# Zhen-Dong/HAWQ

Hardware: NVIDIA H100
Metric: images/sec ResNet-50 W8A8 & W4A4 @batch128, 1/2/4/8xH100; % int-TC roofline (higher is better)
Workload: dtype int8

## Files before the change

hawq_b200/csrc/api.cu:

```cuda
#include <cmath>
#include <cstdarg>
#include <cstdio>
#include <cstring>

#include <cstdlib>

#include "conv_igemm.cuh"
#include "conv_tail.cuh"
#include "elementwise.cuh"
#include "eval_transform.cuh"
#include "mobilenet.cuh"
#include "stem.cuh"

using namespace hawq;

struct hawq_handle {
  int device;
  int sm_count;
  int32_t* status;
};

static thread_local char g_err[512] = "";
static long long g_kernel_count[8] = {0, 0, 0, 0, 0, 0, 0, 0};

namespace hawq {
int fail(int code, const char* fmt, ...) {
  va_list ap;
  va_start(ap, fmt);
  vsnprintf(g_err, sizeof(g_err), fmt, ap);
  va_end(ap);
  return code;
}
}

#define CUDA_TRY(expr)                                                                         \
  do {                                                                                         \
    cudaError_t _e = (expr);                                                                   \
    if (_e != cudaSuccess) return fail(HAWQ_ERR_CUDA, "%s: %s", #expr, cudaGetErrorString(_e)); \
  } while (0)

static int launch_check(const char* what) {
  cudaError_t e = cudaGetLastError();
  if (e != cudaSuccess) return fail(HAWQ_ERR_CUDA, "%s launch: %s", what, cudaGetErrorString(e));
  return HAWQ_OK;
}

static int grid_for(long long work_items, int sm_count) {
  long long blocks = (work_items + 255) / 256;
  const long long cap = (long long)sm_count * 16;
  if (blocks > cap) blocks = cap;
  if (blocks < 1) blocks = 1;
  return (int)blocks;
}

template <class K>
static int set_smem_attr(K* kernel, int smem) {
  CUDA_TRY(cudaFuncSetAttribute(kernel, cudaFuncAttributeMaxDynamicSharedMemorySize, smem));
  CUDA_TRY(cudaFuncSetAttribute(kernel, cudaFuncAttributePreferredSharedMemoryCarveout, cudaSharedmemCarveoutMaxShared));
  return HAWQ_OK;
}
template <int BN, bool A4>
static int set_conv_attr() {
  constexpr int smem = ConvSmem<BN, A4>::TOTAL;
  int rc;
  if ((rc = set_smem_attr(conv_igemm_kernel<BN, A4, FAM_REQUANT>, smem)) || (rc = set_smem_attr(conv_igemm_kernel<BN, A4, FAM_RESIDUAL>, smem)) ||
      (rc = set_smem_attr(conv_igemm_kernel<BN, A4, FAM_REQUANT_CAPPED>, smem)) ||
      (rc = set_smem_attr(conv_igemm_kernel<BN, A4, FAM_STORE>, smem)) ||
      (rc = set_smem_attr(conv_tail_kernel<A4, false>, TailSmem<A4, false>::TOTAL)) ||
      (rc = set_smem_attr(conv_tail_kernel<A4, true>, TailSmem<A4, true>::TOTAL)))
    return rc;
  return HAWQ_OK;
}

static dim3 conv_grid(long long M, int Cout, int BN) { return dim3((unsigned)((M + CONV_BM - 1) / CONV_BM * (Cout / BN)), 1, 1); }

template <int BN, bool A4>
static void launch_conv(const ConvParams& p, cudaStream_t s) {
  const int smem = ConvSmem<BN, A4>::TOTAL;
  const dim3 grid = conv_grid(p.M, p.Cout, BN);
  if (p.mode == HAWQ_EPI_REQUANT && p.relu == 2) conv_igemm_kernel<BN, A4, FAM_REQUANT_CAPPED><<<grid, CONV_THREADS, smem, s>>>(p);
  else if (p.mode == HAWQ_EPI_REQUANT) conv_igemm_kernel<BN, A4, FAM_REQUANT><<<grid, CONV_THREADS, smem, s>>>(p);
  else if (p.mode == HAWQ_EPI_RESIDUAL) conv_igemm_kernel<BN, A4, FAM_RESIDUAL><<<grid, CONV_THREADS, smem, s>>>(p);
  else conv_igemm_kernel<BN, A4, FAM_STORE><<<grid, CONV_THREADS, smem, s>>>(p);
}
template <bool A4, bool DUAL>
static void launch_conv_tail(const ConvParams& p, int sm_count, cudaStream_t s) {
  conv_tail_kernel<A4, DUAL><<<tail_grid(p.Cout, sm_count), CONV_THREADS, TailSmem<A4, DUAL>::TOTAL, s>>>(p);
}

extern "C" {

int hawq_abi_version(void) { return HAWQ_ABI_VERSION; }
const char* hawq_last_error(void) { return g_err; }

static int create_on(int device, hawq_handle** out) {
  CUDA_TRY(cudaSetDevice(device));
  cudaDeviceProp prop;
  CUDA_TRY(cudaGetDeviceProperties(&prop, device));
  if (prop.major != 9 || prop.minor != 0)
    return fail(HAWQ_ERR_UNSUPPORTED, "hawq_create: device sm_%d%d is not Hopper sm_90 (the library is built for sm_90a)", prop.major, prop.minor);
  hawq_handle* h = new hawq_handle();
  h->device = device;
  h->sm_count = prop.multiProcessorCount;
  h->status = nullptr;
  CUDA_TRY(cudaMalloc(&h->status, sizeof(int32_t)));
  CUDA_TRY(cudaMemset(h->status, 0, sizeof(int32_t)));
  int rc;
  CUDA_TRY(cudaFuncSetAttribute(linear_dp4a_kernel, cudaFuncAttributeMaxDynamicSharedMemorySize, linear_smem_bytes(LIN_MAX_K)));
  if ((rc = set_conv_attr<128, false>()) || (rc = set_conv_attr<64, false>()) || (rc = set_conv_attr<128, true>()) ||
      (rc = set_conv_attr<64, true>()))
    return rc;
  *out = h;
  return HAWQ_OK;
}

int hawq_create(int device, hawq_handle** out) {
  if (!out) return fail(HAWQ_ERR_BAD_ARG, "hawq_create: out is null");
  int prev = 0;
  CUDA_TRY(cudaGetDevice(&prev));
  int rc = create_on(device, out);
  cudaSetDevice(prev);
  return rc;
}

int hawq_destroy(hawq_handle* h) {
  if (!h) return HAWQ_OK;
  cudaFree(h->status);
  delete h;
  return HAWQ_OK;
}

int hawq_sm_count(const hawq_handle* h) { return h ? h->sm_count : 0; }

int hawq_reset_status(hawq_handle* h, void* stream) {
  if (!h) return fail(HAWQ_ERR_BAD_ARG, "null handle");
  CUDA_TRY(cudaMemsetAsync(h->status, 0, sizeof(int32_t), (cudaStream_t)stream));
  return HAWQ_OK;
}

int hawq_get_status(hawq_handle* h, void* stream, int32_t* host_flags) {
  if (!h || !host_flags) return fail(HAWQ_ERR_BAD_ARG, "null argument");
  CUDA_TRY(cudaMemcpyAsync(host_flags, h->status, sizeof(int32_t), cudaMemcpyDeviceToHost, (cudaStream_t)stream));
  CUDA_TRY(cudaStreamSynchronize((cudaStream_t)stream));
  return HAWQ_OK;
}

int hawq_copy_status(hawq_handle* h, int32_t* dst, void* stream) {
  if (!h || !dst) return fail(HAWQ_ERR_BAD_ARG, "null argument");
  CUDA_TRY(cudaMemcpyAsync(dst, h->status, sizeof(int32_t), cudaMemcpyDeviceToDevice, (cudaStream_t)stream));
  return HAWQ_OK;
}

static int check_me(const char* fn, const char* what, uint32_t m, int e) {
  return e < 1 || e > 62 || m > 0x80000000u ? fail(HAWQ_ERR_BAD_ARG, "%s: %s dyadic pair out of range (m=%u e=%d)", fn, what, m, e) : HAWQ_OK;
}

static int out_size(int in, int k, int stride, int pad) { return (in + 2 * pad - k) / stride + 1; }

static int check_conv_desc(const char* fn, const hawq_conv_desc* d, int bn) {
  if (d->N < 1 || d->H < 1 || d->W < 1 || d->kh < 1 || d->kw < 1 || d->stride < 1 || d->pad < 0) return fail(HAWQ_ERR_BAD_ARG, "%s: bad geometry", fn);
  if (d->a_bits != 8 && d->a_bits != 4) return fail(HAWQ_ERR_UNSUPPORTED, "%s: a_bits must be 4 or 8", fn);
  if (d->Cin % 64 != 0 || d->Cout % 64 != 0) return fail(HAWQ_ERR_UNSUPPORTED, "%s: Cin (%d) and Cout (%d) must be multiples of 64", fn, d->Cin, d->Cout);
  if (d->Cin < 64 || d->Cout < 64) return fail(HAWQ_ERR_BAD_ARG, "%s: Cin (%d) and Cout (%d) must be at least 64", fn, d->Cin, d->Cout);
  const int Ho = out_size(d->H, d->kh, d->stride, d->pad), Wo = out_size(d->W, d->kw, d->stride, d->pad);
  if (Ho < 1 || Wo < 1) return fail(HAWQ_ERR_BAD_ARG, "%s: empty output", fn);
  const long long M = (long long)d->N * Ho * Wo;
  if (M > 0x7fffff00ll || (long long)d->N * d->H * d->W > 0x7fffff00ll) return fail(HAWQ_ERR_UNSUPPORTED, "%s: too many pixels", fn);
  if ((M + CONV_BM - 1) / CONV_BM * (d->Cout / bn) > 0x7fffffffll) return fail(HAWQ_ERR_UNSUPPORTED, "%s: more than 2^31 - 1 output tiles", fn);
  return HAWQ_OK;
}

static int check_dims(const char* fn, int N, int H, int W, int C, int min_side = 1) {
  return N < 1 || H < min_side || W < min_side || C < 1 ? fail(HAWQ_ERR_BAD_ARG, "%s: bad geometry", fn) : HAWQ_OK;
}

static int check_limits(const char* fn, long long pixels, long long ctas) {
  if (pixels > 0x7fffff00ll) return fail(HAWQ_ERR_UNSUPPORTED, "%s: too many pixels", fn);
  if (ctas > 0x7fffffffll) return fail(HAWQ_ERR_UNSUPPORTED, "%s: more than 2^31 - 1 CTAs", fn);
  return HAWQ_OK;
}

static int check_clamp(const char* fn, int lo, int hi, int bits = 0) {
  if (lo > hi) return fail(HAWQ_ERR_BAD_ARG, "%s: empty clamp range", fn);
  if (bits && (lo < -(1 << (bits - 1)) || hi >= 1 << (bits - 1))) return fail(HAWQ_ERR_BAD_ARG, "%s: clamp must fit int%d", fn, bits);
  return HAWQ_OK;
}

static int check_low(const char* fn, int low_bits, uint32_t low_m, int low_e, const void* out_low) {
  if (low_bits != 0 && low_bits != 4 && low_bits != 8) return fail(HAWQ_ERR_BAD_ARG, "%s: low_bits must be 0/4/8", fn);
  if (!low_bits) return HAWQ_OK;
  if (!out_low) return fail(HAWQ_ERR_BAD_ARG, "%s: low_bits set but out_low is null", fn);
  return check_me(fn, "low-bit copy", low_m, low_e);
}

static int check_residual(const char* fn, const hawq_epilogue_desc* ep, const void* res, const hawq_chan* res_chan, const void* y,
                          const void* out_low) {
  if (!res) return fail(HAWQ_ERR_BAD_ARG, "%s: RESIDUAL needs res", fn);
  if (ep->res_kind != 0 && ep->res_kind != 1) return fail(HAWQ_ERR_BAD_ARG, "%s: res_kind must be 0/1", fn);
  if (ep->res_kind == 1 && !res_chan) return fail(HAWQ_ERR_BAD_ARG, "%s: res_kind 1 needs res_chan", fn);
  if (ep->res_kind == 0 && ep->res_bits != 16 && ep->res_bits != 32) return fail(HAWQ_ERR_BAD_ARG, "%s: res_bits must be 16/32", fn);
  if (int rc = ep->res_kind == 0 ? check_me(fn, "residual", ep->res_m, ep->res_e) : HAWQ_OK) return rc;
  if (ep->y_bits != 0 && ep->y_bits != 16 && ep->y_bits != 32) return fail(HAWQ_ERR_BAD_ARG, "%s: y_bits must be 0/16/32", fn);
  if (ep->y_bits == 16 && !ep->relu) return fail(HAWQ_ERR_BAD_ARG, "%s: uint16 residual stream requires relu", fn);
  if (ep->y_bits && !y) return fail(HAWQ_ERR_BAD_ARG, "%s: y_bits set but the stream pointer is null", fn);
  if (!ep->y_bits && !ep->low_bits) return fail(HAWQ_ERR_BAD_ARG, "%s: RESIDUAL with no output", fn);
  return check_low(fn, ep->low_bits, ep->low_m, ep->low_e, out_low);
}

static void set_bias_window(ConvParams& p, int a_bits) {
  long long bound = (long long)p.K * (a_bits == 4 ? 15 * 128 : 128 * 128);
  if (bound > 2147483648ll) bound = 2147483648ll;
  p.bias_lo = (int)(bound - 2147483648ll);
  p.bias_hi = (int)(2147483647ll - bound);
}

static ConvParams conv_params(const hawq_handle* h, const hawq_conv_desc& d, const void* x, const int8_t* w, const hawq_chan* chan,
                              void* out, bool depthwise = false) {
  ConvParams p;
  memset(&p, 0, sizeof(p));
  p.x = (const uint8_t*)x; p.w = w; p.chan = chan; p.out = out; p.status = h->status;
  p.N = d.N; p.H = d.H; p.W = d.W; p.Cin = d.Cin; p.Cout = d.Cout; p.KH = d.kh; p.KW = d.kw; p.stride = d.stride; p.pad = d.pad;
  p.Ho = out_size(d.H, d.kh, d.stride, d.pad); p.Wo = out_size(d.W, d.kw, d.stride, d.pad);
  p.M = (int)((long long)d.N * p.Ho * p.Wo); p.K = d.kh * d.kw * (depthwise ? 1 : d.Cin);
  p.cin_chunks = d.Cin / 64; p.x_pix_bytes = d.Cin * d.a_bits / 8;
  set_bias_window(p, d.a_bits);
  return p;
}

static void set_epilogue(ConvParams& p, const hawq_epilogue_desc& ep, bool writes_low) {
  p.mode = ep.mode; p.relu = ep.relu; p.out_bits = ep.out_bits; p.lo = ep.clamp_lo; p.hi = ep.clamp_hi;
  p.res_kind = ep.res_kind; p.res_bits = ep.res_bits; p.res_m = ep.res_m; p.res_e = ep.res_e;
  p.y_bits = ep.y_bits; p.low_bits = ep.low_bits; p.low_m = ep.low_m; p.low_e = ep.low_e; p.low_lo = ep.low_lo; p.low_hi = ep.low_hi;
  p.cout_store = ep.cout_store;
  const bool residual = ep.mode == HAWQ_EPI_RESIDUAL, scalar_res = residual && ep.res_kind == 0;
  const bool low_over_one = writes_low && ep.low_bits != 0 && !dyadic_is_fast(ep.low_m, ep.low_e);
  p.scalar_over_one = (scalar_res && !dyadic_is_fast(ep.res_m, ep.res_e)) || low_over_one;
  p.scalar_unchecked = (scalar_res && !dyadic_is_wide(ep.res_m, ep.res_e)) || low_over_one;
  p.check_ovf = residual && (ep.flags & (HAWQ_EP_RATIOS_LE_ONE | HAWQ_EP_RATIOS_LE_2P20)) != 0;
}

static int persistent_ctas(long long tiles, int sm_count) { return (int)(tiles < 4LL * sm_count ? tiles : 4LL * sm_count); }

int hawq_conv2d(hawq_handle* h, const hawq_conv_desc* d, const hawq_epilogue_desc* ep, const void* x, const int8_t* w,
                const hawq_chan* chan, const void* res, const hawq_chan* res_chan, const float* fscale, void* out,
                void* out_low, void* stream) {
  if (!h || !d || !ep || !x || !w || !chan) return fail(HAWQ_ERR_BAD_ARG, "hawq_conv2d: null argument");
  const bool bn128 = (d->Cout % 128 == 0);
  if (int rc = check_conv_desc(__func__, d, bn128 ? 128 : 64)) return rc;
  switch (ep->mode) {
    case HAWQ_EPI_REQUANT:
      if (!out) return fail(HAWQ_ERR_BAD_ARG, "hawq_conv2d: REQUANT needs out");
      if (ep->out_bits != 4 && ep->out_bits != 8 && ep->out_bits != 16 && ep->out_bits != 32)
        return fail(HAWQ_ERR_BAD_ARG, "hawq_conv2d: out_bits must be 4/8/16/32");
      if (int rc = check_clamp(__func__, ep->clamp_lo, ep->clamp_hi)) return rc;
      break;
    case HAWQ_EPI_RESIDUAL:
      if (int rc = check_residual(__func__, ep, res, res_chan, out, out_low)) return rc;
      break;
    case HAWQ_EPI_RAW_I32:
      if (!out) return fail(HAWQ_ERR_BAD_ARG, "hawq_conv2d: RAW_I32 needs out");
      break;
    case HAWQ_EPI_DEQUANT_F32:
      if (!out || !fscale) return fail(HAWQ_ERR_BAD_ARG, "hawq_conv2d: DEQUANT_F32 needs out and fscale");
      if (ep->cout_store < 1 || ep->cout_store > d->Cout) return fail(HAWQ_ERR_BAD_ARG, "hawq_conv2d: bad cout_store");
      break;
    default:
      return fail(HAWQ_ERR_BAD_ARG, "hawq_conv2d: unknown epilogue mode %d", ep->mode);
  }

  ConvParams p = conv_params(h, *d, x, w, chan, out);
  p.res = res; p.res_chan = res_chan; p.fscale = fscale; p.out_low = out_low;
  set_epilogue(p, *ep, ep->mode == HAWQ_EPI_RESIDUAL);
  ++g_kernel_count[0];
  cudaStream_t s = (cudaStream_t)stream;
  const bool tail = ep->mode == HAWQ_EPI_RESIDUAL && d->kh == 1 && d->kw == 1 && d->stride == 1 && d->pad == 0 && ep->res_kind == 0 &&
                    ep->res_bits == 16 && ep->y_bits == 16;
  if (tail) {
    if (d->a_bits == 8) launch_conv_tail<false, false>(p, h->sm_count, s);
    else launch_conv_tail<true, false>(p, h->sm_count, s);
  } else if (d->a_bits == 8) {
    if (bn128) launch_conv<128, false>(p, s);
    else launch_conv<64, false>(p, s);
  } else {
    if (bn128) launch_conv<128, true>(p, s);
    else launch_conv<64, true>(p, s);
  }
  return launch_check("conv_igemm");
}

int hawq_conv2d_dual(hawq_handle* h, const hawq_conv_desc* d, const hawq_epilogue_desc* ep, const void* x, const int8_t* w,
                     const hawq_chan* chan, const hawq_conv_desc* d2, const void* x2, const int8_t* w2, const hawq_chan* chan2,
                     void* out, void* out_low, void* stream) {
  if (!h || !d || !ep || !x || !w || !chan || !d2 || !x2 || !w2 || !chan2 || !out) return fail(HAWQ_ERR_BAD_ARG, "hawq_conv2d_dual: null argument");
  if (d->kh != 1 || d->kw != 1 || d->stride != 1 || d->pad != 0 || d2->kh != 1 || d2->kw != 1 || d2->pad != 0 || d2->stride < 1)
    return fail(HAWQ_ERR_UNSUPPORTED, "hawq_conv2d_dual: both convolutions must be 1x1 without padding (main stride 1)");
  int rc;
  if ((rc = check_conv_desc(__func__, d, 64))) return rc;
  if (d2->a_bits != d->a_bits || d2->Cout != d->Cout) return fail(HAWQ_ERR_UNSUPPORTED, "hawq_conv2d_dual: a_bits and Cout must be equal");
  if (d2->N != d->N || out_size(d2->H, 1, d2->stride, 0) != d->H || out_size(d2->W, 1, d2->stride, 0) != d->W)
    return fail(HAWQ_ERR_BAD_ARG, "hawq_conv2d_dual: the two convolutions have different output grids");
  if ((rc = check_conv_desc(__func__, d2, 64))) return rc;
  if (d->w_layout != 1 || d2->w_layout != 1) return fail(HAWQ_ERR_UNSUPPORTED, "hawq_conv2d_dual: weights must carry the re-tiled copy (w_layout 1)");
  if (ep->mode != HAWQ_EPI_RESIDUAL || !ep->relu || ep->y_bits != 16) return fail(HAWQ_ERR_UNSUPPORTED, "hawq_conv2d_dual: RESIDUAL + relu + uint16 stream only");
  if ((rc = check_low(__func__, ep->low_bits, ep->low_m, ep->low_e, out_low))) return rc;
  if (ep->low_bits && !dyadic_is_fast(ep->low_m, ep->low_e)) return fail(HAWQ_ERR_UNSUPPORTED, "hawq_conv2d_dual: low-bit ratio outside the fast range");
  if (!(ep->flags & (HAWQ_EP_RATIOS_LE_ONE | HAWQ_EP_RATIOS_LE_2P20))) return fail(HAWQ_ERR_UNSUPPORTED, "hawq_conv2d_dual: needs a ratio-range promise (flags)");

  ++g_kernel_count[4];
  ConvParams p = conv_params(h, *d, x, w, chan, out);
  const ConvParams id = conv_params(h, *d2, x2, w2, chan2, nullptr);
  p.x2 = id.x; p.w2 = id.w; p.H2 = id.H; p.W2 = id.W; p.stride2 = id.stride; p.cin_chunks2 = id.cin_chunks; p.x2_pix_bytes = id.x_pix_bytes;
  p.res_chan = chan2; p.out_low = out_low;
  const hawq_epilogue_desc e = {HAWQ_EPI_RESIDUAL, 1, 0, 0, 0, 1, 32, 0, 0, 16, ep->low_bits, ep->low_m, ep->low_e, ep->low_lo, ep->low_hi, 0, ep->flags};
  set_epilogue(p, e, true);

  cudaStream_t s = (cudaStream_t)stream;
  if (d->a_bits == 8) launch_conv_tail<false, true>(p, h->sm_count, s);
  else launch_conv_tail<true, true>(p, h->sm_count, s);
  return launch_check("conv_dual");
}

int hawq_conv2d_i8(hawq_handle* h, const hawq_conv_desc* d, const hawq_epilogue_desc* ep, const void* x,
                   const int8_t* w, const hawq_chan* chan, const void* res, const hawq_chan* res_chan,
                   const float* fscale, void* out, void* out_low, void* stream) {
  if (d && d->a_bits != 8) return fail(HAWQ_ERR_BAD_ARG, "hawq_conv2d_i8: a_bits must be 8");
  return hawq_conv2d(h, d, ep, x, w, chan, res, res_chan, fscale, out, out_low, stream);
}

int hawq_conv2d_i4(hawq_handle* h, const hawq_conv_desc* d, const hawq_epilogue_desc* ep, const void* x,
                   const int8_t* w, const hawq_chan* chan, const void* res, const hawq_chan* res_chan,
                   const float* fscale, void* out, void* out_low, void* stream) {
  if (d && d->a_bits != 4) return fail(HAWQ_ERR_BAD_ARG, "hawq_conv2d_i4: a_bits must be 4");
  return hawq_conv2d(h, d, ep, x, w, chan, res, res_chan, fscale, out, out_low, stream);
}

int hawq_linear_i8(hawq_handle* h, int32_t N, int32_t K, int32_t Cout, int32_t Cout_pad, const int8_t* x,
                   const int8_t* w, const hawq_chan* chan, const float* fscale, float* out, void* stream) {
  if (Cout < 1 || Cout > Cout_pad) return fail(HAWQ_ERR_BAD_ARG, "hawq_linear_i8: bad Cout/Cout_pad");
  if (!h || !x || !w || !chan || !fscale || !out || N < 1 || K < 1) return fail(HAWQ_ERR_BAD_ARG, "hawq_linear_i8: null argument or empty shape");
  static const bool dp4a_enabled = [] { const char* e = getenv("HAWQ_B200_LINEAR_DP4A"); return !(e && e[0] == '0'); }();
  if (dp4a_enabled && K % LIN_SLAB == 0 && K <= LIN_MAX_K && Cout_pad % LIN_CH == 0 && N <= 65535 * LIN_ROWS) {
    const dim3 grid((unsigned)(Cout_pad / LIN_CH), (unsigned)((N + LIN_ROWS - 1) / LIN_ROWS), 1);
    linear_dp4a_kernel<<<grid, 256, linear_smem_bytes(K), (cudaStream_t)stream>>>(x, w, chan, fscale, out, N, K, Cout);
    return launch_check("linear_dp4a");
  }
  const hawq_conv_desc d = {N, 1, 1, K, Cout_pad, 1, 1, 1, 0, 8, 0};
  hawq_epilogue_desc ep = {};
  ep.mode = HAWQ_EPI_DEQUANT_F32;
  ep.cout_store = Cout;
  return hawq_conv2d(h, &d, &ep, x, w, chan, nullptr, nullptr, fscale, out, nullptr, stream);
}

static ConvParams stem_params(hawq_handle* h, int N, int H, int W, const int8_t* x, const int8_t* w, const hawq_chan* chan,
                              const hawq_epilogue_desc& ep, void* out, void* out_low) {
  ConvParams p = conv_params(h, {N, H, W, 3, 64, 7, 7, 2, 3, 8, 0}, x, w, chan, out);
  p.out_low = out_low;
  set_epilogue(p, ep, true);
  return p;
}

int hawq_stem_conv_i8(hawq_handle* h, int32_t N, int32_t H, int32_t W, const int8_t* x, const int8_t* w,
                      const hawq_chan* chan, int32_t clamp_lo, int32_t clamp_hi, int16_t* out, void* stream) {
// ... 238 lines not shown
```

hawq_b200/csrc/conv_igemm.cuh:

```cuda
#pragma once
#include <type_traits>

#include "common.cuh"
#include "wgmma.cuh"

namespace hawq {

struct ConvParams {
  const uint8_t* x;
  const int8_t* w;
  const hawq_chan* chan;
  const void* res;
  const hawq_chan* res_chan;
  const float* fscale;
  void* out;
  void* out_low;
  int32_t* status;
  int N, H, W, Cin, Cout, KH, KW, stride, pad, Ho, Wo, M, K;
  int cin_chunks;
  int x_pix_bytes;
  int mode, relu, out_bits, lo, hi;
  int res_kind, res_bits;
  uint32_t res_m;
  int res_e;
// ... 125 lines not shown
    if (checked && count) {
      const double q = t - kMagic;
      ovf |= q > 2147483647.0 || q < -2147483648.0;
    }
    return __double2loint(t);
  }
};
struct RqExact {
  bool checked;
  bool ovf = false;
  __device__ static int32_t acc_bias(int32_t acc, double, int32_t bias) { return sat_add(acc, bias); }
  __device__ static int32_t of_i32(int32_t v) { return v; }
  __device__ static int32_t of_u16(uint32_t u) { return (int32_t)u; }
  __device__ int32_t term(int32_t v, double, uint32_t m, int32_t e, bool count) {
    const long long q = rhe_requant64(v, m, e);
    if (checked && count) ovf |= q > 2147483647ll || q < -2147483648ll;
    return sat_i32(q);
  }
};

struct RqPolicy {
  bool over_one;
  bool unchecked;
  bool clamped;
};

template <int BN, bool RESIDUAL, bool CAPS = false>
__device__ RqPolicy load_channel_block(const ConvParams& p, int n0, const ChanSmem<BN>& cs) {
  int over_one = p.scalar_over_one, unchecked = p.scalar_unchecked, bias_out = 0;
  const int tid = threadIdx.x;
  if (tid < BN) {
    hawq_chan c = p.chan[n0 + tid];
    if (CAPS) c.reserved = p.relu == 2 ? min(p.hi, c.reserved) : p.hi;
    cs.chan[tid] = c;
    cs.M[tid] = dyadic_to_double(c.m, c.e);
    cs.Cb[tid] = 4503601774854144.0 - (double)c.bias;
    bias_out = c.bias < p.bias_lo || c.bias > p.bias_hi;
    over_one |= !dyadic_is_fast(c.m, c.e);
    unchecked |= !dyadic_is_wide(c.m, c.e);
    if (RESIDUAL && p.res_kind == 1) {
      const hawq_chan rc = p.res_chan[n0 + tid];
      cs.rc[tid] = rc;
      cs.M1[tid] = dyadic_to_double(rc.m, rc.e);
      over_one |= !dyadic_is_fast(rc.m, rc.e);
      unchecked |= !dyadic_is_wide(rc.m, rc.e);
    }
  }
  RqPolicy pol;
  pol.over_one = __syncthreads_or(over_one) != 0;
  pol.unchecked = __syncthreads_or(unchecked) != 0;
  pol.clamped = __syncthreads_or(bias_out) != 0;
  return pol;
}

template <bool RESIDUAL, class F>
__device__ __forceinline__ void with_rq(const RqPolicy& pol, const ConvParams& p, F&& f) {
  const bool fp64 = !pol.over_one || (RESIDUAL && p.check_ovf && !pol.unchecked);
  if (!fp64) f(RqExact{RESIDUAL && p.check_ovf != 0});
  else if (pol.clamped) f(RqFp64<true>{RESIDUAL && pol.over_one});
  else f(RqFp64<false>{RESIDUAL && pol.over_one});
}

template <class Rq>
__device__ __forceinline__ int32_t residual_y(Rq& rq, int32_t res_term, int32_t acc, double cb, const int4& c, double M, bool ok,
                                              int32_t relu_floor) {
  return max(sat_add(res_term, rq.term(rq.acc_bias(acc, cb, c.x), M, c.y, c.z, ok)), relu_floor);
}
template <class Rq>
__device__ __forceinline__ int32_t residual_low(Rq& rq, int32_t y, double low_M, const ConvParams& p) {
  return clampi(rq.term(rq.of_i32(y), low_M, p.low_m, p.low_e, false), p.low_lo, p.low_hi);
}
__device__ __forceinline__ uint32_t stream16_pair(int32_t y0, int32_t y1, bool ok, int& ymax) {
  if (ok) ymax = max(ymax, max(y0, y1));
  return (uint32_t)min(y0, 65535) | ((uint32_t)min(y1, 65535) << 16);
}
__device__ __forceinline__ void residual_flags(const ConvParams& p, int ymax, bool ovf) {
  if (ymax > 65535) atomicOr(p.status, HAWQ_FLAG_RESIDUAL_OVERFLOW);
  if (ovf) atomicOr(p.status, HAWQ_FLAG_REQUANT_OVERFLOW);
}
__device__ __forceinline__ void stage_low_pair(uint8_t* s, int pitch, int row, int col, int q0, int q1) {
  *reinterpret_cast<uint16_t*>(s + row * pitch + col) = (uint16_t)__byte_perm(q0, q1, 0x0040);
}

__device__ __forceinline__ void copy_out_rows(const uint8_t* s, int s_pitch, uint8_t* g, size_t g_pitch, int row_bytes, int m0, int M) {
  const int cpr = row_bytes / 16;
  for (int id = threadIdx.x; id < CONV_BM * cpr; id += blockDim.x) {
    const int row = id / cpr, j = id - row * cpr;
    if (m0 + row < M)
      *reinterpret_cast<int4*>(g + (size_t)(m0 + row) * g_pitch + j * 16) = *reinterpret_cast<const int4*>(s + row * s_pitch + j * 16);
  }
}
template <int BN>
__device__ __forceinline__ void copy_out_low(const uint8_t* s, int pitch, uint8_t* gout, int bits, int m0, int n0, int M, int Cout) {
  if (bits == 8) {
    copy_out_rows(s, pitch, gout + n0, (size_t)Cout, BN, m0, M);
  } else {
    constexpr int CPR = BN / 32;
    for (int id = threadIdx.x; id < CONV_BM * CPR; id += blockDim.x) {
      const int row = id / CPR, j = id % CPR;
      if (m0 + row < M) {
        const uint4 a = *reinterpret_cast<const uint4*>(s + row * pitch + j * 32);
        const uint4 b = *reinterpret_cast<const uint4*>(s + row * pitch + j * 32 + 16);
        uint4 o;
        o.x = pack_nibbles8(a.x, a.y);
        o.y = pack_nibbles8(a.z, a.w);
        o.z = pack_nibbles8(b.x, b.y);
        o.w = pack_nibbles8(b.z, b.w);
        *reinterpret_cast<uint4*>(gout + (((size_t)(m0 + row) * Cout + n0 + j * 32) >> 1)) = o;
      }
    }
  }
}

struct ConvGeom {
  const uint8_t* x;
  const int8_t* w;
  int H, W, stride, pad, KH, KW, cin_chunks, x_pix_bytes, K;
};

template <int BN, bool A4, int FAM>
__global__ void __launch_bounds__(CONV_THREADS, 2) conv_igemm_kernel(const ConvParams p) {
  using S = ConvSmem<BN, A4>;
  constexpr int BM = CONV_BM, STAGES = CONV_STAGES;
  constexpr int A_ROW = S::A_ROW, A_CH = S::A_CH, A_ROWS_PER_PASS = S::A_ROWS_PER_PASS, A_PASSES = S::A_PASSES;
  constexpr int NT = S::NT, NACC = S::NACC;
  constexpr int B_PASSES = BN / 64;

  extern __shared__ __align__(1024) uint8_t smem[];
  uint8_t* sA = smem;
  uint8_t* sB = smem + STAGES * S::A_STAGE;
  const ChanSmem<BN> cs(smem + S::CHAN_OFF);
  const hawq_chan* sChan = cs.chan;
  const double* sM = cs.M;
  const double* sM1 = cs.M1;
  const hawq_chan* sResChan = cs.rc;
  const double* sCb = cs.Cb;

  const int tid = threadIdx.x;
  const AccFrag fr(tid);
  const int nblk = p.Cout / BN;
  const int m0 = (int)(blockIdx.x / nblk) * BM;
  const int n0 = (int)(blockIdx.x % nblk) * BN;

  constexpr bool REQ = FAM == FAM_REQUANT || FAM == FAM_REQUANT_CAPPED;
  const RqPolicy pol = load_channel_block<BN, FAM == FAM_RESIDUAL, FAM == FAM_REQUANT_CAPPED>(p, n0, cs);

  int32_t acc[NACC];

  const int res_es = (FAM == FAM_RESIDUAL) ? ((p.res_kind == 1 || p.res_bits == 32) ? 4 : 2) : 0;
  const int res_pitch = tile_pitch(BN, res_es);
  uint8_t* sRes = smem + (res_es == 2 ? S::RES16_OFF : S::RES32_OFF);

  auto load_res = [&]() {
    if constexpr (FAM == FAM_RESIDUAL) load_res_tile<BN>(sRes, p, res_es, m0, n0);
  };
  const bool prefetch_res = res_es == 2;

  auto gemm = [&](const ConvGeom& gm, bool with_res) {
#pragma unroll
    for (int i = 0; i < NACC; ++i) acc[i] = 0;
    const int a_ch = tid % A_CH;
    int a_hi0[A_PASSES], a_wi0[A_PASSES], a_pix[A_PASSES];
    bool a_ok[A_PASSES];
#pragma unroll
    for (int i = 0; i < A_PASSES; ++i) {
      const int row = tid / A_CH + i * A_ROWS_PER_PASS;
      const int m = m0 + row;
      a_ok[i] = m < p.M;
      const int mm = a_ok[i] ? m : 0;
      const int n = mm / (p.Ho * p.Wo);
      const int r = mm - n * (p.Ho * p.Wo);
      const int ho = r / p.Wo, wo = r - ho * p.Wo;
      a_hi0[i] = ho * gm.stride - gm.pad;
      a_wi0[i] = wo * gm.stride - gm.pad;
      a_pix[i] = n * gm.H * gm.W;
    }
    const int b_ch = tid & 3, b_row = tid >> 2;
    const int KT = gm.KH * gm.KW * gm.cin_chunks;
    int ld_c = 0, ld_kw = 0, ld_kh = 0, ld_kt = 0;

    auto load_tile = [&](int stage) {
      const uint32_t a_base = smem_u32(sA + stage * S::A_STAGE);
#pragma unroll
      for (int i = 0; i < A_PASSES; ++i) {
        const int row = tid / A_CH + i * A_ROWS_PER_PASS;
        const int hi = a_hi0[i] + ld_kh, wi = a_wi0[i] + ld_kw;
        const bool v = a_ok[i] && (unsigned)hi < (unsigned)gm.H && (unsigned)wi < (unsigned)gm.W;
        const uint8_t* src = gm.x;
        if (v) src = gm.x + (size_t)(a_pix[i] + hi * gm.W + wi) * gm.x_pix_bytes + ld_c * A_ROW + a_ch * 16;
        cp_async_16(a_base + swz<A_ROW>(row, a_ch), src, v ? 16 : 0);
      }
      const uint32_t b_base = smem_u32(sB + stage * S::B_STAGE);
#pragma unroll
      for (int i = 0; i < B_PASSES; ++i) {
        const int row = b_row + i * 64;
        const int8_t* src = gm.w + (size_t)(n0 + row) * gm.K + ld_kt * 64 + b_ch * 16;
        cp_async_16(b_base + swz<64>(row, b_ch), src, 16);
      }
      ++ld_kt;
      if (++ld_c == gm.cin_chunks) {
        ld_c = 0;
        if (++ld_kw == gm.KW) { ld_kw = 0; ++ld_kh; }
      }
    };

#pragma unroll
    for (int s = 0; s < STAGES - 1; ++s) {
      if (s < KT) load_tile(s);
      if (s == STAGES - 2 && with_res) load_res();
      cp_async_commit();
    }

    for (int kt = 0; kt < KT; ++kt) {
      cp_async_wait<STAGES - 2>();
      fence_proxy_async_smem();
      __syncthreads();
      if (kt + STAGES - 1 < KT) load_tile((kt + STAGES - 1) % STAGES);
      cp_async_commit();

      const int stage = kt % STAGES;
      mma_ktile<BN, A4>(acc, smem_u32(sA + stage * S::A_STAGE), smem_u32(sB + stage * S::B_STAGE));
    }
    cp_async_wait<0>();
    __syncthreads();
  };

  gemm(ConvGeom{p.x, p.w, p.H, p.W, p.stride, p.pad, p.KH, p.KW, p.cin_chunks, p.x_pix_bytes, p.K}, prefetch_res);

  if (res_es == 4) {
    load_res();
    cp_async_commit();
    cp_async_wait<0>();
    __syncthreads();
  }
  const bool y_staged = res_es != 0 && p.y_bits == res_es * 8;
  const int y_es = p.y_bits / 8;
  const int y_pitch = tile_pitch(BN, y_es);
  uint8_t* sY = sRes;

  uint8_t* sOut = smem;
  const bool stage_low = (REQ && p.out_bits <= 8) || (FAM == FAM_RESIDUAL && p.low_bits != 0);
  const int stage_bits = REQ ? p.out_bits : p.low_bits;

  auto put_low = [&](int row, int col, int q0, int q1) { stage_low_pair(sOut, S::OUT_PITCH, row, col, q0, q1); };
  auto put_y = [&](int row, int col, bool ok, int y0, int y1, int& ymax) {
    const uint32_t y16 = p.y_bits == 16 ? stream16_pair(y0, y1, ok, ymax) : 0u;
    if (!y_staged && !ok) return;
    uint8_t* dst = y_staged ? sY + row * y_pitch + col * y_es
                            : reinterpret_cast<uint8_t*>(p.out) + ((size_t)(m0 + row) * p.Cout + n0 + col) * y_es;
    if (p.y_bits == 16) *reinterpret_cast<uint32_t*>(dst) = y16;
    else if (p.y_bits == 32) *reinterpret_cast<int2*>(dst) = make_int2(y0, y1);
  };

  auto epilogue = [&](auto rq, auto low_out) {
    if constexpr (REQ) {
      const int lo = p.relu ? min(max(p.lo, 0), p.hi) : p.lo;
#pragma unroll
      for (int ni = 0; ni < NT; ++ni) {
        const int col = fr.col(ni);
        const int4 c0 = *reinterpret_cast<const int4*>(&sChan[col]);
        const int4 c1 = *reinterpret_cast<const int4*>(&sChan[col + 1]);
        const double2 M = *reinterpret_cast<const double2*>(&sM[col]);
        const double2 Cb = *reinterpret_cast<const double2*>(&sCb[col]);
        const int hi0 = FAM == FAM_REQUANT_CAPPED ? c0.w : p.hi, hi1 = FAM == FAM_REQUANT_CAPPED ? c1.w : p.hi;
#pragma unroll
        for (int hf = 0; hf < 2; ++hf) {
          const int row = fr.row(hf);
          const int q0 = clampi(rq.term(rq.acc_bias(acc[acc_idx(ni, hf)], Cb.x, c0.x), M.x, c0.y, c0.z, false), lo, hi0);
          const int q1 = clampi(rq.term(rq.acc_bias(acc[acc_idx(ni, hf) + 1], Cb.y, c1.x), M.y, c1.y, c1.z, false), lo, hi1);
          if constexpr (decltype(low_out)::value) {
            put_low(row, col, q0, q1);
          } else if (m0 + row < p.M) {
            uint8_t* dst = reinterpret_cast<uint8_t*>(p.out) + ((size_t)(m0 + row) * p.Cout + n0 + col) * (p.out_bits / 8);
            if (p.out_bits == 16) *reinterpret_cast<uint32_t*>(dst) = (uint32_t)(q0 & 0xFFFF) | ((uint32_t)q1 << 16);
            else *reinterpret_cast<int2*>(dst) = make_int2(q0, q1);
          }
        }
      }
    } else {
      const double res_M = dyadic_to_double(p.res_m, p.res_e), low_M = dyadic_to_double(p.low_m, p.low_e);
      const int relu_floor = p.relu ? 0 : (int)0x80000000;
      int ymax = 0;
#pragma unroll
      for (int ni = 0; ni < NT; ++ni) {
        const int col = fr.col(ni);
        const int4 c0 = *reinterpret_cast<const int4*>(&sChan[col]);
        const int4 c1 = *reinterpret_cast<const int4*>(&sChan[col + 1]);
        const double2 M = *reinterpret_cast<const double2*>(&sM[col]);
        const double2 Cb = *reinterpret_cast<const double2*>(&sCb[col]);
        double2 M1 = make_double2(res_M, res_M);
        uint2 m1 = make_uint2(p.res_m, p.res_m);
        int2 e1 = make_int2(p.res_e, p.res_e);
        if (p.res_kind == 1) {
          M1 = *reinterpret_cast<const double2*>(&sM1[col]);
          m1 = make_uint2(sResChan[col].m, sResChan[col + 1].m);
          e1 = make_int2(sResChan[col].e, sResChan[col + 1].e);
        }
#pragma unroll
        for (int hf = 0; hf < 2; ++hf) {
          const int row = fr.row(hf);
          const bool ok = m0 + row < p.M;
          const uint8_t* rptr = sRes + row * res_pitch + col * res_es;
          decltype(rq.of_i32(0)) r0, r1;
          if (res_es == 2) {
            const uint32_t pr = *reinterpret_cast<const uint32_t*>(rptr);
            r0 = rq.of_u16(pr & 0xFFFFu);
            r1 = rq.of_u16(pr >> 16);
          } else {
            const int2 pr = *reinterpret_cast<const int2*>(rptr);
            r0 = rq.of_i32(pr.x);
            r1 = rq.of_i32(pr.y);
          }
          const int y0 = residual_y(rq, rq.term(r0, M1.x, m1.x, e1.x, ok), acc[acc_idx(ni, hf)], Cb.x, c0, M.x, ok, relu_floor);
          const int y1 = residual_y(rq, rq.term(r1, M1.y, m1.y, e1.y, ok), acc[acc_idx(ni, hf) + 1], Cb.y, c1, M.y, ok, relu_floor);
          put_y(row, col, ok, y0, y1, ymax);
          if (p.low_bits != 0) put_low(row, col, residual_low(rq, y0, low_M, p), residual_low(rq, y1, low_M, p));
        }
      }
      residual_flags(p, ymax, rq.ovf);
    }
  };

  if constexpr (FAM == FAM_STORE) {
#pragma unroll
    for (int ni = 0; ni < NT; ++ni) {
      const int col = fr.col(ni);
      const int b0 = sChan[col].bias, b1 = sChan[col + 1].bias;
#pragma unroll
      for (int hf = 0; hf < 2; ++hf) {
        const int m = m0 + fr.row(hf);
        if (m >= p.M) continue;
        const int32_t v0 = sat_add(acc[acc_idx(ni, hf)], b0), v1 = sat_add(acc[acc_idx(ni, hf) + 1], b1);
        if (p.mode == HAWQ_EPI_RAW_I32) {
          *reinterpret_cast<int2*>(reinterpret_cast<int32_t*>(p.out) + (size_t)m * p.Cout + n0 + col) = make_int2(v0, v1);
        } else {
          float* o = reinterpret_cast<float*>(p.out) + (size_t)m * p.cout_store;
          const int c = n0 + col;
          if (c < p.cout_store) o[c] = __fmul_rn((float)v0, p.fscale[c]);
          if (c + 1 < p.cout_store) o[c + 1] = __fmul_rn((float)v1, p.fscale[c + 1]);
        }
      }
    }
  } else {
    auto run = [&](auto low_out) { with_rq<FAM == FAM_RESIDUAL>(pol, p, [&](auto rq) { epilogue(rq, low_out); }); };
    if (REQ && p.out_bits <= 8) run(std::true_type{});
    else run(std::false_type{});
  }

  if (y_staged || stage_low) __syncthreads();
  if (y_staged)
    copy_out_rows(sY, y_pitch, reinterpret_cast<uint8_t*>(p.out) + (size_t)n0 * y_es, (size_t)p.Cout * y_es, BN * y_es, m0, p.M);
  if (stage_low)
    copy_out_low<BN>(sOut, S::OUT_PITCH, reinterpret_cast<uint8_t*>(REQ ? p.out : p.out_low), stage_bits, m0, n0, p.M, p.Cout);
}

}
```

hawq_b200/csrc/wgmma.cuh:

```cuda
#pragma once
#include "common.cuh"

namespace hawq {

__device__ __forceinline__ constexpr int acc_idx(int j, int h) { return j * 4 + h * 2; }
struct AccFrag {
  int warp, g, t;
  __device__ explicit AccFrag(int tid) : warp(tid >> 5), g((tid & 31) >> 2), t(tid & 3) {}
  __device__ int row(int h) const { return warp * 16 + h * 8 + g; }
  __device__ int col(int j) const { return j * 8 + 2 * t; }
};

__device__ __forceinline__ uint64_t wgmma_desc_sw64(uint32_t smem_addr) {
  return (uint64_t)((smem_addr >> 4) & 0x3FFFu) | ((uint64_t)1 << 16) | ((uint64_t)(512 >> 4) << 32) | ((uint64_t)2 << 62);
}
__device__ __forceinline__ void wgmma_fence() { asm volatile("wgmma.fence.sync.aligned;" ::: "memory"); }
__device__ __forceinline__ void wgmma_commit() { asm volatile("wgmma.commit_group.sync.aligned;" ::: "memory"); }
__device__ __forceinline__ void wgmma_wait_all() { asm volatile("wgmma.wait_group.sync.aligned 0;" ::: "memory"); }
__device__ __forceinline__ void fence_proxy_async_smem() { asm volatile("fence.proxy.async.shared::cta;" ::: "memory"); }
template <int N>
__device__ __forceinline__ void fence_operands(int32_t (&d)[N]) {
#pragma unroll
  for (int i = 0; i < N; ++i) asm volatile("" : "+r"(d[i])::"memory");
}

__device__ __forceinline__ void wgmma_ss_n64_s8(int32_t (&d)[32], uint64_t adesc, uint64_t bdesc) {
  asm volatile(
      "wgmma.mma_async.sync.aligned.m64n64k32.s32.s8.s8 "
      "{%0, %1, %2, %3, %4, %5, %6, %7, %8, %9, %10, %11, %12, %13, %14, %15, %16, %17, %18, %19, %20, %21, %22, %23, %24, %25, %26, %27, %28, %29, %30, %31}, "
      "%32, %33, 1;"
      : "+r"(d[0]), "+r"(d[1]), "+r"(d[2]), "+r"(d[3]), "+r"(d[4]), "+r"(d[5]), "+r"(d[6]), "+r"(d[7]), "+r"(d[8]), "+r"(d[9]), "+r"(d[10]), "+r"(d[11]), "+r"(d[12]), "+r"(d[13]), "+r"(d[14]), "+r"(d[15]), "+r"(d[16]), "+r"(d[17]), "+r"(d[18]), "+r"(d[19]), "+r"(d[20]), "+r"(d[21]), "+r"(d[22]), "+r"(d[23]), "+r"(d[24]), "+r"(d[25]), "+r"(d[26]), "+r"(d[27]), "+r"(d[28]), "+r"(d[29]), "+r"(d[30]), "+r"(d[31])
      : "l"(adesc), "l"(bdesc)
      : "memory");
}

__device__ __forceinline__ void wgmma_rs_n64_u8(int32_t (&d)[32], const uint32_t (&a)[4], uint64_t bdesc) {
  asm volatile(
      "wgmma.mma_async.sync.aligned.m64n64k32.s32.u8.s8 "
      "{%0, %1, %2, %3, %4, %5, %6, %7, %8, %9, %10, %11, %12, %13, %14, %15, %16, %17, %18, %19, %20, %21, %22, %23, %24, %25, %26, %27, %28, %29, %30, %31}, "
      "{%32, %33, %34, %35}, %36, 1;"
      : "+r"(d[0]), "+r"(d[1]), "+r"(d[2]), "+r"(d[3]), "+r"(d[4]), "+r"(d[5]), "+r"(d[6]), "+r"(d[7]), "+r"(d[8]), "+r"(d[9]), "+r"(d[10]), "+r"(d[11]), "+r"(d[12]), "+r"(d[13]), "+r"(d[14]), "+r"(d[15]), "+r"(d[16]), "+r"(d[17]), "+r"(d[18]), "+r"(d[19]), "+r"(d[20]), "+r"(d[21]), "+r"(d[22]), "+r"(d[23]), "+r"(d[24]), "+r"(d[25]), "+r"(d[26]), "+r"(d[27]), "+r"(d[28]), "+r"(d[29]), "+r"(d[30]), "+r"(d[31])
      : "r"(a[0]), "r"(a[1]), "r"(a[2]), "r"(a[3]), "l"(bdesc)
      : "memory");
}

__device__ __forceinline__ void wgmma_ss_n128_s8(int32_t (&d)[64], uint64_t adesc, uint64_t bdesc) {
  asm volatile(
      "wgmma.mma_async.sync.aligned.m64n128k32.s32.s8.s8 "
      "{%0, %1, %2, %3, %4, %5, %6, %7, %8, %9, %10, %11, %12, %13, %14, %15, %16, %17, %18, %19, %20, %21, %22, %23, %24, %25, %26, %27, %28, %29, %30, %31, %32, %33, %34, %35, %36, %37, %38, %39, %40, %41, %42, %43, %44, %45, %46, %47, %48, %49, %50, %51, %52, %53, %54, %55, %56, %57, %58, %59, %60, %61, %62, %63}, "
      "%64, %65, 1;"
      : "+r"(d[0]), "+r"(d[1]), "+r"(d[2]), "+r"(d[3]), "+r"(d[4]), "+r"(d[5]), "+r"(d[6]), "+r"(d[7]), "+r"(d[8]), "+r"(d[9]), "+r"(d[10]), "+r"(d[11]), "+r"(d[12]), "+r"(d[13]), "+r"(d[14]), "+r"(d[15]), "+r"(d[16]), "+r"(d[17]), "+r"(d[18]), "+r"(d[19]), "+r"(d[20]), "+r"(d[21]), "+r"(d[22]), "+r"(d[23]), "+r"(d[24]), "+r"(d[25]), "+r"(d[26]), "+r"(d[27]), "+r"(d[28]), "+r"(d[29]), "+r"(d[30]), "+r"(d[31]), "+r"(d[32]), "+r"(d[33]), "+r"(d[34]), "+r"(d[35]), "+r"(d[36]), "+r"(d[37]), "+r"(d[38]), "+r"(d[39]), "+r"(d[40]), "+r"(d[41]), "+r"(d[42]), "+r"(d[43]), "+r"(d[44]), "+r"(d[45]), "+r"(d[46]), "+r"(d[47]), "+r"(d[48]), "+r"(d[49]), "+r"(d[50]), "+r"(d[51]), "+r"(d[52]), "+r"(d[53]), "+r"(d[54]), "+r"(d[55]), "+r"(d[56]), "+r"(d[57]), "+r"(d[58]), "+r"(d[59]), "+r"(d[60]), "+r"(d[61]), "+r"(d[62]), "+r"(d[63])
      : "l"(adesc), "l"(bdesc)
      : "memory");
}

__device__ __forceinline__ void wgmma_rs_n128_u8(int32_t (&d)[64], const uint32_t (&a)[4], uint64_t bdesc) {
  asm volatile(
      "wgmma.mma_async.sync.aligned.m64n128k32.s32.u8.s8 "
      "{%0, %1, %2, %3, %4, %5, %6, %7, %8, %9, %10, %11, %12, %13, %14, %15, %16, %17, %18, %19, %20, %21, %22, %23, %24, %25, %26, %27, %28, %29, %30, %31, %32, %33, %34, %35, %36, %37, %38, %39, %40, %41, %42, %43, %44, %45, %46, %47, %48, %49, %50, %51, %52, %53, %54, %55, %56, %57, %58, %59, %60, %61, %62, %63}, "
      "{%64, %65, %66, %67}, %68, 1;"
      : "+r"(d[0]), "+r"(d[1]), "+r"(d[2]), "+r"(d[3]), "+r"(d[4]), "+r"(d[5]), "+r"(d[6]), "+r"(d[7]), "+r"(d[8]), "+r"(d[9]), "+r"(d[10]), "+r"(d[11]), "+r"(d[12]), "+r"(d[13]), "+r"(d[14]), "+r"(d[15]), "+r"(d[16]), "+r"(d[17]), "+r"(d[18]), "+r"(d[19]), "+r"(d[20]), "+r"(d[21]), "+r"(d[22]), "+r"(d[23]), "+r"(d[24]), "+r"(d[25]), "+r"(d[26]), "+r"(d[27]), "+r"(d[28]), "+r"(d[29]), "+r"(d[30]), "+r"(d[31]), "+r"(d[32]), "+r"(d[33]), "+r"(d[34]), "+r"(d[35]), "+r"(d[36]), "+r"(d[37]), "+r"(d[38]), "+r"(d[39]), "+r"(d[40]), "+r"(d[41]), "+r"(d[42]), "+r"(d[43]), "+r"(d[44]), "+r"(d[45]), "+r"(d[46]), "+r"(d[47]), "+r"(d[48]), "+r"(d[49]), "+r"(d[50]), "+r"(d[51]), "+r"(d[52]), "+r"(d[53]), "+r"(d[54]), "+r"(d[55]), "+r"(d[56]), "+r"(d[57]), "+r"(d[58]), "+r"(d[59]), "+r"(d[60]), "+r"(d[61]), "+r"(d[62]), "+r"(d[63])
      : "r"(a[0]), "r"(a[1]), "r"(a[2]), "r"(a[3]), "l"(bdesc)
      : "memory");
}

template <int N>
__device__ __forceinline__ void wgmma_ss(int32_t (&d)[N / 2], uint64_t adesc, uint64_t bdesc) {
  if constexpr (N == 128) wgmma_ss_n128_s8(d, adesc, bdesc);
  else wgmma_ss_n64_s8(d, adesc, bdesc);
}
template <int N>
__device__ __forceinline__ void wgmma_rs(int32_t (&d)[N / 2], const uint32_t (&a)[4], uint64_t bdesc) {
  if constexpr (N == 128) wgmma_rs_n128_u8(d, a, bdesc);
  else wgmma_rs_n64_u8(d, a, bdesc);
}

}
```

Before: 29410.

## Add persistent halo-tiled 3x3 conv kernel for 64-channel stride-1 layers

```diff
diff --git a/hawq_b200/csrc/api.cu b/hawq_b200/csrc/api.cu
--- a/hawq_b200/csrc/api.cu
+++ b/hawq_b200/csrc/api.cu
@@ -5,6 +5,7 @@
 
 #include <cstdlib>
 
+#include "conv3x3.cuh"
 #include "conv_igemm.cuh"
 #include "conv_tail.cuh"
 #include "elementwise.cuh"
@@ -82,6 +83,14 @@
   else if (p.mode == HAWQ_EPI_REQUANT) conv_igemm_kernel<BN, A4, FAM_REQUANT><<<grid, CONV_THREADS, smem, s>>>(p);
   else if (p.mode == HAWQ_EPI_RESIDUAL) conv_igemm_kernel<BN, A4, FAM_RESIDUAL><<<grid, CONV_THREADS, smem, s>>>(p);
   else conv_igemm_kernel<BN, A4, FAM_STORE><<<grid, CONV_THREADS, smem, s>>>(p);
+}
+static int conv3x3_grid(int Cout, int sm_count) {
+  const int nblk = Cout / C3_BN, per = 2 * sm_count / nblk;
+  return (per > 1 ? per : 1) * nblk;
+}
+static bool conv3x3_fills(const hawq_conv_desc& d, int sm_count) {
+  const long long tiles = ((long long)d.N * (d.H + 2) * (d.W + 2) + C3_BM - 1) / C3_BM;
+  return tiles * (d.Cout / C3_BN) >= conv3x3_grid(d.Cout, sm_count);
 }
 template <bool A4, bool DUAL>
 static void launch_conv_tail(const ConvParams& p, int sm_count, cudaStream_t s) {
@@ -108,7 +117,7 @@
   int rc;
   CUDA_TRY(cudaFuncSetAttribute(linear_dp4a_kernel, cudaFuncAttributeMaxDynamicSharedMemorySize, linear_smem_bytes(LIN_MAX_K)));
   if ((rc = set_conv_attr<128, false>()) || (rc = set_conv_attr<64, false>()) || (rc = set_conv_attr<128, true>()) ||
-      (rc = set_conv_attr<64, true>()))
+      (rc = set_conv_attr<64, true>()) || (rc = set_smem_attr(conv3x3_kernel, Conv3x3Smem::TOTAL)))
     return rc;
   *out = h;
   return HAWQ_OK;
@@ -275,9 +284,14 @@
   cudaStream_t s = (cudaStream_t)stream;
   const bool tail = ep->mode == HAWQ_EPI_RESIDUAL && d->kh == 1 && d->kw == 1 && d->stride == 1 && d->pad == 0 && ep->res_kind == 0 &&
                     ep->res_bits == 16 && ep->y_bits == 16;
+  const bool c3 = ep->mode == HAWQ_EPI_REQUANT && ep->relu != 2 && ep->out_bits <= 8 && d->kh == 3 && d->kw == 3 && d->stride == 1 &&
+                  d->pad == 1 && d->a_bits == 8 && d->Cin == 64 && d->W <= C3_MAX_W &&
+                  (long long)d->N * (d->H + 2) * (d->W + 2) <= 0x7fffff00ll - C3_HALO && conv3x3_fills(*d, h->sm_count);
   if (tail) {
     if (d->a_bits == 8) launch_conv_tail<false, false>(p, h->sm_count, s);
     else launch_conv_tail<true, false>(p, h->sm_count, s);
+  } else if (c3) {
+    conv3x3_kernel<<<conv3x3_grid(p.Cout, h->sm_count), CONV_THREADS, Conv3x3Smem::TOTAL, s>>>(p);
   } else if (d->a_bits == 8) {
     if (bn128) launch_conv<128, false>(p, s);
     else launch_conv<64, false>(p, s);
diff --git a/hawq_b200/csrc/conv3x3.cuh b/hawq_b200/csrc/conv3x3.cuh
--- /dev/null
+++ b/hawq_b200/csrc/conv3x3.cuh
@@ -0,0 +1,123 @@
+#pragma once
+#include "conv_igemm.cuh"
+
+namespace hawq {
+
+constexpr int C3_BM = 256;
+constexpr int C3_BN = 64;
+constexpr int C3_HALO = 512;
+constexpr int C3_MAX_W = (C3_HALO - C3_BM - 2) / 2 - 2;
+
+struct Conv3x3Smem {
+  static constexpr int B_TAP = C3_BN * 64;
+  static constexpr int HALO = C3_HALO * 64;
+  static constexpr int HALO_OFF = 9 * B_TAP;
+  static constexpr int OUT_PITCH = ConvRing<C3_BN, false>::OUT_PITCH;
+  static constexpr int ROWS_OFF = HALO_OFF + 2 * HALO;
+  static constexpr int CHAN_OFF = ROWS_OFF + C3_BM * 4;
+  static constexpr int TOTAL = CHAN_OFF + ChanSmem<C3_BN>::BYTES;
+  static_assert(B_TAP % 512 == 0 && HALO_OFF % 512 == 0 && HALO % 512 == 0, "SWIZZLE_64B tiles must stay 512-B aligned");
+  static_assert(C3_BM * OUT_PITCH <= HALO, "the staging tile must fit in a consumed halo stage");
+  static_assert(2 * (TOTAL + 1024) <= 228 * 1024, "two CTAs per SM must fit in shared memory");
+};
+
+struct HaloRows {
+  const int* rows;
+  __device__ bool ok(int r) const { return rows[r] >= 0; }
+  __device__ int at(int r) const { return rows[r]; }
+};
+
+__global__ void __launch_bounds__(CONV_THREADS, 2) conv3x3_kernel(const ConvParams p) {
+  using S = Conv3x3Smem;
+  constexpr int BN = C3_BN;
+  extern __shared__ __align__(1024) uint8_t smem[];
+  int* sRow = reinterpret_cast<int*>(smem + S::ROWS_OFF);
+  const ChanSmem<BN> cs(smem + S::CHAN_OFF);
+
+  const int tid = threadIdx.x, wg = tid >> 7;
+  const AccFrag fr(tid);
+  const int nblk = p.Cout / BN;
+  const int n0 = (int)(blockIdx.x % nblk) * BN;
+  const int rt0 = (int)(blockIdx.x / nblk), rstep = (int)(gridDim.x / nblk);
+  const int Wp = p.W + 2, PP = (p.H + 2) * Wp;
+  const int nrt = (p.N * PP + C3_BM - 1) / C3_BM;
+  if (rt0 >= nrt) return;
+  const int T = (nrt - rt0 + rstep - 1) / rstep;
+  const int halo = C3_BM + 2 * Wp + 2;
+
+  const RqPolicy pol = load_channel_block<BN, false>(p, n0, cs);
+
+  const uint32_t bb = smem_u32(smem);
+  for (int id = tid; id < 9 * BN * 4; id += CONV_THREADS) {
+    const int j = id & 3, row = (id >> 2) % BN, tap = (id >> 2) / BN;
+    cp_async_16(bb + tap * S::B_TAP + swz<64>(row, j), p.w + (size_t)(n0 + row) * p.K + tap * 64 + j * 16, 16);
+  }
+  auto issue = [&](int t) {
+    if (t < T) {
+      const uint32_t hb = smem_u32(smem + S::HALO_OFF + (t & 1) * S::HALO);
+      const int ch = tid & 3;
+      int px = tid >> 2;
+      const int q = (rt0 + t * rstep) * C3_BM + px;
+      int n = q / PP;
+      int r = (q - n * PP) / Wp;
+      int c = q - n * PP - r * Wp;
+      for (; px < halo; px += CONV_THREADS / 4) {
+        const bool v = n < p.N && (unsigned)(r - 1) < (unsigned)p.H && (unsigned)(c - 1) < (unsigned)p.W;
+        const uint8_t* src = v ? p.x + ((size_t)(n * p.H + r - 1) * p.W + c - 1) * 64 + ch * 16 : p.x;
+        cp_async_16(hb + swz<64>(px, ch), src, v ? 16 : 0);
+        for (c += CONV_THREADS / 4; c >= Wp; c -= Wp)
+          if (++r == p.H + 2) { r = 0; ++n; }
+      }
+    }
+    cp_async_commit();
+  };
+
+  int32_t acc[2][BN / 2];
+  issue(0);
+  issue(1);
+  with_rq<false>(pol, p, [&](auto rq) {
+    for (int t = 0; t < T; ++t) {
+#pragma unroll
+      for (int i = 0; i < BN / 2; ++i) acc[0][i] = acc[1][i] = 0;
+      cp_async_wait<1>();
+      fence_proxy_async_smem();
+      __syncthreads();
+      uint8_t* st = smem + S::HALO_OFF + (t & 1) * S::HALO;
+      const uint32_t hb = smem_u32(st) + wg * 64 * 64;
+      wgmma_fence();
+#pragma unroll
+      for (int tap = 0; tap < 9; ++tap) {
+        const uint32_t a_tap = hb + ((tap / 3) * Wp + tap % 3) * 64;
+#pragma unroll
+        for (int ks = 0; ks < 2; ++ks) {
+          const uint64_t bdesc = wgmma_desc_sw64(bb + tap * S::B_TAP + ks * 32);
+#pragma unroll
+          for (int h = 0; h < 2; ++h)
+            wgmma_ss<BN>(acc[h], wgmma_desc_sw64_at(a_tap + h * 128 * 64 + ks * 32), bdesc);
+        }
+      }
+      wgmma_commit();
+      wgmma_wait_all();
+      fence_operands(acc[0]);
+      fence_operands(acc[1]);
+
+      __syncthreads();
+      {
+        static_assert(CONV_THREADS == C3_BM, "one tile row per thread");
+        const int q = (rt0 + t * rstep) * C3_BM + tid;
+        const int n = q / PP, r = (q - n * PP) / Wp, c = q - n * PP - r * Wp;
+        sRow[tid] = n < p.N && r < p.H && c < p.W ? (n * p.H + r) * p.W + c : -1;
+      }
+      auto put = [&](int row, int col, int q0, int q1) { stage_low_pair(st, S::OUT_PITCH, row, col, q0, q1); };
+      requant_frag<BN, false>(rq, acc[0], cs, fr, 0, p, put);
+      requant_frag<BN, false>(rq, acc[1], cs, fr, 128, p, put);
+      __syncthreads();
+      copy_out_low<BN, C3_BM>(st, S::OUT_PITCH, reinterpret_cast<uint8_t*>(p.out), p.out_bits, n0, p.Cout, HaloRows{sRow});
+      __syncthreads();
+      issue(t + 2);
+    }
+  });
+  cp_async_wait<0>();
+}
+
+}
diff --git a/hawq_b200/csrc/conv_igemm.cuh b/hawq_b200/csrc/conv_igemm.cuh
--- a/hawq_b200/csrc/conv_igemm.cuh
+++ b/hawq_b200/csrc/conv_igemm.cuh
@@ -231,23 +231,33 @@
   *reinterpret_cast<uint16_t*>(s + row * pitch + col) = (uint16_t)__byte_perm(q0, q1, 0x0040);
 }
 
+struct TileRows {
+  int m0, M;
+  __device__ bool ok(int r) const { return m0 + r < M; }
+  __device__ int at(int r) const { return m0 + r; }
+};
+
+template <int ROWS, class RowMap>
+__device__ __forceinline__ void copy_out_rows(const uint8_t* s, int s_pitch, uint8_t* g, size_t g_pitch, int row_bytes, RowMap out_row) {
+  const int cpr = row_bytes / 16;
+  for (int id = threadIdx.x; id < ROWS * cpr; id += blockDim.x) {
+    const int row = id / cpr, j = id - row * cpr;
+    if (out_row.ok(row))
+      *reinterpret_cast<int4*>(g + (size_t)out_row.at(row) * g_pitch + j * 16) = *reinterpret_cast<const int4*>(s + row * s_pitch + j * 16);
+  }
+}
 __device__ __forceinline__ void copy_out_rows(const uint8_t* s, int s_pitch, uint8_t* g, size_t g_pitch, int row_bytes, int m0, int M) {
-  const int cpr = row_bytes / 16;
-  for (int id = threadIdx.x; id < CONV_BM * cpr; id += blockDim.x) {
-    const int row = id / cpr, j = id - row * cpr;
-    if (m0 + row < M)
-      *reinterpret_cast<int4*>(g + (size_t)(m0 + row) * g_pitch + j * 16) = *reinterpret_cast<const int4*>(s + row * s_pitch + j * 16);
-  }
-}
-template <int BN>
-__device__ __forceinline__ void copy_out_low(const uint8_t* s, int pitch, uint8_t* gout, int bits, int m0, int n0, int M, int Cout) {
+  copy_out_rows<CONV_BM>(s, s_pitch, g, g_pitch, row_bytes, TileRows{m0, M});
+}
+template <int BN, int ROWS, class RowMap>
+__device__ __forceinline__ void copy_out_low(const uint8_t* s, int pitch, uint8_t* gout, int bits, int n0, int Cout, RowMap out_row) {
   if (bits == 8) {
-    copy_out_rows(s, pitch, gout + n0, (size_t)Cout, BN, m0, M);
+    copy_out_rows<ROWS>(s, pitch, gout + n0, (size_t)Cout, BN, out_row);
   } else {
     constexpr int CPR = BN / 32;
-    for (int id = threadIdx.x; id < CONV_BM * CPR; id += blockDim.x) {
+    for (int id = threadIdx.x; id < ROWS * CPR; id += blockDim.x) {
       const int row = id / CPR, j = id % CPR;
-      if (m0 + row < M) {
+      if (out_row.ok(row)) {
         const uint4 a = *reinterpret_cast<const uint4*>(s + row * pitch + j * 32);
         const uint4 b = *reinterpret_cast<const uint4*>(s + row * pitch + j * 32 + 16);
         uint4 o;
@@ -255,8 +265,33 @@
         o.y = pack_nibbles8(a.z, a.w);
         o.z = pack_nibbles8(b.x, b.y);
         o.w = pack_nibbles8(b.z, b.w);
-        *reinterpret_cast<uint4*>(gout + (((size_t)(m0 + row) * Cout + n0 + j * 32) >> 1)) = o;
+        *reinterpret_cast<uint4*>(gout + (((size_t)out_row.at(row) * Cout + n0 + j * 32) >> 1)) = o;
       }
+    }
+  }
+}
+template <int BN>
+__device__ __forceinline__ void copy_out_low(const uint8_t* s, int pitch, uint8_t* gout, int bits, int m0, int n0, int M, int Cout) {
+  copy_out_low<BN, CONV_BM>(s, pitch, gout, bits, n0, Cout, TileRows{m0, M});
+}
+
+template <int BN, bool CAPPED, class Rq, class Put>
+__device__ __forceinline__ void requant_frag(Rq& rq, const int32_t (&acc)[BN / 2], const ChanSmem<BN>& cs, const AccFrag& fr, int row0,
+                                             const ConvParams& p, Put&& put) {
+  const int lo = p.relu ? min(max(p.lo, 0), p.hi) : p.lo;
+#pragma unroll
+  for (int ni = 0; ni < BN / 8; ++ni) {
+    const int col = fr.col(ni);
+    const int4 c0 = *reinterpret_cast<const int4*>(&cs.chan[col]);
+    const int4 c1 = *reinterpret_cast<const int4*>(&cs.chan[col + 1]);
+    const double2 M = *reinterpret_cast<const double2*>(&cs.M[col]);
+    const double2 Cb = *reinterpret_cast<const double2*>(&cs.Cb[col]);
+    const int hi0 = CAPPED ? c0.w : p.hi, hi1 = CAPPED ? c1.w : p.hi;
+#pragma unroll
+    for (int hf = 0; hf < 2; ++hf) {
+      const int q0 = clampi(rq.term(rq.acc_bias(acc[acc_idx(ni, hf)], Cb.x, c0.x), M.x, c0.y, c0.z, false), lo, hi0);
+      const int q1 = clampi(rq.term(rq.acc_bias(acc[acc_idx(ni, hf) + 1], Cb.y, c1.x), M.y, c1.y, c1.z, false), lo, hi1);
+      put(row0 + fr.row(hf), col, q0, q1);
     }
   }
 }
@@ -403,29 +438,15 @@
 
   auto epilogue = [&](auto rq, auto low_out) {
     if constexpr (REQ) {
-      const int lo = p.relu ? min(max(p.lo, 0), p.hi) : p.lo;
-#pragma unroll
-      for (int ni = 0; ni < NT; ++ni) {
-        const int col = fr.col(ni);
-        const int4 c0 = *reinterpret_cast<const int4*>(&sChan[col]);
-        const int4 c1 = *reinterpret_cast<const int4*>(&sChan[col + 1]);
-        const double2 M = *reinterpret_cast<const double2*>(&sM[col]);
-        const double2 Cb = *reinterpret_cast<const double2*>(&sCb[col]);
-        const int hi0 = FAM == FAM_REQUANT_CAPPED ? c0.w : p.hi, hi1 = FAM == FAM_REQUANT_CAPPED ? c1.w : p.hi;
-#pragma unroll
-        for (int hf = 0; hf < 2; ++hf) {
-          const int row = fr.row(hf);
-          const int q0 = clampi(rq.term(rq.acc_bias(acc[acc_idx(ni, hf)], Cb.x, c0.x), M.x, c0.y, c0.z, false), lo, hi0);
-          const int q1 = clampi(rq.term(rq.acc_bias(acc[acc_idx(ni, hf) + 1], Cb.y, c1.x), M.y, c1.y, c1.z, false), lo, hi1);
-          if constexpr (decltype(low_out)::value) {
-            put_low(row, col, q0, q1);
-          } else if (m0 + row < p.M) {
-            uint8_t* dst = reinterpret_cast<uint8_t*>(p.out) + ((size_t)(m0 + row) * p.Cout + n0 + col) * (p.out_bits / 8);
-            if (p.out_bits == 16) *reinterpret_cast<uint32_t*>(dst) = (uint32_t)(q0 & 0xFFFF) | ((uint32_t)q1 << 16);
-            else *reinterpret_cast<int2*>(dst) = make_int2(q0, q1);
-          }
+      requant_frag<BN, FAM == FAM_REQUANT_CAPPED>(rq, acc, cs, fr, 0, p, [&](int row, int col, int q0, int q1) {
+        if constexpr (decltype(low_out)::value) {
+          put_low(row, col, q0, q1);
+        } else if (m0 + row < p.M) {
+          uint8_t* dst = reinterpret_cast<uint8_t*>(p.out) + ((size_t)(m0 + row) * p.Cout + n0 + col) * (p.out_bits / 8);
+          if (p.out_bits == 16) *reinterpret_cast<uint32_t*>(dst) = (uint32_t)(q0 & 0xFFFF) | ((uint32_t)q1 << 16);
+          else *reinterpret_cast<int2*>(dst) = make_int2(q0, q1);
         }
-      }
+      });
     } else {
       const double res_M = dyadic_to_double(p.res_m, p.res_e), low_M = dyadic_to_double(p.low_m, p.low_e);
       const int relu_floor = p.relu ? 0 : (int)0x80000000;
diff --git a/hawq_b200/csrc/wgmma.cuh b/hawq_b200/csrc/wgmma.cuh
--- a/hawq_b200/csrc/wgmma.cuh
+++ b/hawq_b200/csrc/wgmma.cuh
@@ -13,6 +13,9 @@
 
 __device__ __forceinline__ uint64_t wgmma_desc_sw64(uint32_t smem_addr) {
   return (uint64_t)((smem_addr >> 4) & 0x3FFFu) | ((uint64_t)1 << 16) | ((uint64_t)(512 >> 4) << 32) | ((uint64_t)2 << 62);
+}
+__device__ __forceinline__ uint64_t wgmma_desc_sw64_at(uint32_t smem_addr) {
+  return wgmma_desc_sw64(smem_addr);
 }
 __device__ __forceinline__ void wgmma_fence() { asm volatile("wgmma.fence.sync.aligned;" ::: "memory"); }
 __device__ __forceinline__ void wgmma_commit() { asm volatile("wgmma.commit_group.sync.aligned;" ::: "memory"); }
```

After: 30050 (median of 6 runs). 1.02x the previous value.
